# Madhudorai/encodec-pytorch

Measured on AMD Instinct MI355X. Metric: audio-seconds/sec EnCodec24k train step, batch 32x1s, higher is better.
Workload: dtype f32; 1 GPU; config 3: 24 kHz mono full GAN (MS-STFT disc + Balancer); global_batch=32, parallelism=dp1

## Files before the change

encodec-pytorch_amd/csrc/resblock.hip:

```cpp
#include "common.h"
#include "prof.h"

namespace {

typedef float f32x4v __attribute__((ext_vector_type(4)));
ENCX_DEV f32x4v mfma16(float a, float b, f32x4v c) { return __builtin_amdgcn_mfma_f32_16x16x4f32(a, b, c, 0, 0, 0); }

constexpr int TT = 64;
constexpr int XF = 80;
constexpr int XW = 67;

template <int C>
struct Rb {
    static constexpr int HD = C / 2;
    static constexpr int CG = C == 64 ? 2 : 1;
    static constexpr int NT = 256 * CG;
    static constexpr int SLAB = C * C + C * HD + HD * 3 * C + C + HD;
};

struct RbArgs {
    const float* x;
    const float* w1;
    const float* b1;
    const float* w2;
    const float* b2;
    const float* ws;
    const float* bs;
    float* h;
    float* y;
    const float* dy;
    float* dx;
    float* dh;
    float* slab;
    int B, T, NT;
};

ENCX_DEV void st4(float* row, int t, int T, f32x4v v) {
    if (t + 4 <= T) {
        *(f32x4u*)(row + t) = (f32x4u){v[0], v[1], v[2], v[3]};
    } else {
#pragma unroll
        for (int i = 0; i < 4; ++i)
            if (t + i < T) row[t + i] = v[i];
    }
}
ENCX_DEV f32x4v ld4(const float* row, int t, int T) {
    if (t + 4 <= T) return ld4u(row + t);
    f32x4v v;
#pragma unroll
    for (int i = 0; i < 4; ++i) v[i] = t + i < T ? row[t + i] : 0.f;
    return v;
}
ENCX_DEV int reflect_clamp(int t, int T) { return t < 0 ? -t : (t < T ? t : T - 1); }
typedef __amdgpu_buffer_rsrc_t rsrc_t;
ENCX_DEV rsrc_t rsrc(const float* base, int64_t n) {
    return __builtin_amdgcn_make_buffer_rsrc((void*)base, (short)0, (int)(n * sizeof(float)), 0x00020000);
}
ENCX_DEV float bload(rsrc_t r, int voff, int soff) {
    return __builtin_bit_cast(float, __builtin_amdgcn_raw_buffer_load_b32(r, voff, soff, 0));
}

template <int C>
__global__ __launch_bounds__(Rb<C>::NT) void rb_fwd_kernel(RbArgs a) {
    constexpr int HD = C / 2, CG = Rb<C>::CG, NT = Rb<C>::NT, N1 = HD / 16 / CG, N2 = C / 16 / CG;
    extern __shared__ float sm[];
    float* xs = sm;
    float* es = xs + C * XF;
    float* hs = es + C * XF;
    const int tid = threadIdx.x, lane = tid & 63, wv = tid >> 6, lc = lane & 15, lk = lane >> 4;
    const int m0 = 16 * (wv & 3), g = wv >> 2;
    float bw1[3][C / 4][N1], bw2[HD / 4][N2], bws[C / 4][N2], b1v[N1], bov[N2];
#pragma unroll
    for (int n = 0; n < N1; ++n) {
        const int j = (g * N1 + n) * 16 + lc;
        b1v[n] = a.b1[j];
#pragma unroll
        for (int k = 0; k < 3; ++k)
#pragma unroll
            for (int c4 = 0; c4 < C / 4; ++c4) bw1[k][c4][n] = a.w1[((4 * c4 + lk) * 3 + k) * HD + j];
    }
#pragma unroll
    for (int n = 0; n < N2; ++n) {
        const int o = (g * N2 + n) * 16 + lc;
        bov[n] = a.b2[o] + a.bs[o];
#pragma unroll
        for (int j4 = 0; j4 < HD / 4; ++j4) bw2[j4][n] = a.w2[(4 * j4 + lk) * C + o];
#pragma unroll
        for (int c4 = 0; c4 < C / 4; ++c4) bws[c4][n] = a.ws[(4 * c4 + lk) * C + o];
    }
    const int T = a.T, ntiles = a.B * a.NT;
    constexpr int NW = NT / 64, PR = C / NW;
    float pf[PR], pfh = 0.f;
    const int hc = tid >> 1, hp = TT + (tid & 1);
    auto fetch = [&](int tile) {
        const int b = tile / a.NT, t0 = (tile - b * a.NT) * TT;
        const rsrc_t rx = rsrc(a.x + (int64_t)b * C * T, (int64_t)C * T);
        const int vo = (wv * T + reflect_clamp(t0 - 2 + lane, T)) * 4;
#pragma unroll
        for (int u = 0; u < PR; ++u) pf[u] = bload(rx, vo, u * NW * T * 4);
        if (tid < 2 * C) pfh = bload(rx, (hc * T + reflect_clamp(t0 - 2 + hp, T)) * 4, 0);
    };
    if ((int)blockIdx.x < ntiles) fetch(blockIdx.x);
    for (int tile = blockIdx.x; tile < ntiles; tile += gridDim.x) {
        const int b = tile / a.NT, t0 = (tile - b * a.NT) * TT;
        __syncthreads();
#pragma unroll
        for (int u = 0; u < PR; ++u) {
            xs[(wv + NW * u) * XF + lane] = pf[u];
            es[(wv + NW * u) * XF + lane] = elu(pf[u]);
        }
        if (tid < 2 * C) {
            xs[hc * XF + hp] = pfh;
            es[hc * XF + hp] = elu(pfh);
        }
        __syncthreads();
        if (tile + (int)gridDim.x < ntiles) fetch(tile + gridDim.x);
        f32x4v acc1[N1];
#pragma unroll
        for (int n = 0; n < N1; ++n) acc1[n] = (f32x4v){0.f, 0.f, 0.f, 0.f};
#pragma unroll
        for (int k = 0; k < 3; ++k)
#pragma unroll
            for (int c4 = 0; c4 < C / 4; ++c4) {
                const float av = es[(4 * c4 + lk) * XF + m0 + lc + k];
#pragma unroll
                for (int n = 0; n < N1; ++n) acc1[n] = mfma16(av, bw1[k][c4][n], acc1[n]);
            }
        const int tq = t0 + m0 + 4 * lk;
#pragma unroll
        for (int n = 0; n < N1; ++n) {
            const int j = (g * N1 + n) * 16 + lc;
            f32x4v hv, ev;
#pragma unroll
            for (int i = 0; i < 4; ++i) {
                hv[i] = acc1[n][i] + b1v[n];
                ev[i] = elu(hv[i]);
            }
            *(f32x4v*)(hs + j * XF + m0 + 4 * lk) = ev;
            if (a.h) st4(a.h + ((int64_t)b * HD + j) * T, tq, T, hv);
        }
        __syncthreads();
        f32x4v acc2[N2];
#pragma unroll
        for (int n = 0; n < N2; ++n) acc2[n] = (f32x4v){0.f, 0.f, 0.f, 0.f};
#pragma unroll
        for (int j4 = 0; j4 < HD / 4; ++j4) {
            const float av = hs[(4 * j4 + lk) * XF + m0 + lc];
#pragma unroll
            for (int n = 0; n < N2; ++n) acc2[n] = mfma16(av, bw2[j4][n], acc2[n]);
        }
#pragma unroll
        for (int c4 = 0; c4 < C / 4; ++c4) {
            const float av = xs[(4 * c4 + lk) * XF + m0 + lc + 2];
#pragma unroll
            for (int n = 0; n < N2; ++n) acc2[n] = mfma16(av, bws[c4][n], acc2[n]);
        }
#pragma unroll
        for (int n = 0; n < N2; ++n) {
            const int o = (g * N2 + n) * 16 + lc;
            st4(a.y + ((int64_t)b * C + o) * T, tq, T, acc2[n] + bov[n]);
        }
    }
}

template <int C>
__global__ __launch_bounds__(Rb<C>::NT) void rb_dgrad_kernel(RbArgs a) {
    constexpr int HD = C / 2, CG = Rb<C>::CG, NT = Rb<C>::NT, NH = HD / 16 / CG, NX = C / 16 / CG;
    constexpr int TPO = NT / (2 * HD), U = C / TPO;
    static_assert(TPO == 8, "halo reduction assumes 8 lanes per output");
    extern __shared__ float sm[];
    float* dys = sm;
    float* dhs = dys + C * XF;
    const int tid = threadIdx.x, lane = tid & 63, wv = tid >> 6, lc = lane & 15, lk = lane >> 4;
    const int m0 = 16 * (wv & 3), g = wv >> 2;
    float bh[C / 4][NH], bs[C / 4][NX], b3[3][HD / 4][NX];
#pragma unroll
    for (int n = 0; n < NH; ++n) {
        const int j = (g * NH + n) * 16 + lc;
#pragma unroll
        for (int o4 = 0; o4 < C / 4; ++o4) bh[o4][n] = a.w2[j * C + 4 * o4 + lk];
    }
#pragma unroll
    for (int n = 0; n < NX; ++n) {
        const int c = (g * NX + n) * 16 + lc;
#pragma unroll
        for (int o4 = 0; o4 < C / 4; ++o4) bs[o4][n] = a.ws[c * C + 4 * o4 + lk];
#pragma unroll
        for (int k = 0; k < 3; ++k)
#pragma unroll
            for (int j4 = 0; j4 < HD / 4; ++j4) b3[k][j4][n] = a.w1[(c * 3 + k) * HD + 4 * j4 + lk];
    }
    const int hq = tid / TPO, hr = tid - hq * TPO, hj = hq >> 1, hp = TT + (hq & 1);
    float hw[U];
#pragma unroll
    for (int u = 0; u < U; ++u) hw[u] = a.w2[hj * C + hr * U + u];
    const int T = a.T, ntiles = a.B * a.NT;
    constexpr int NW = NT / 64, PR = C / NW;
    float pf[PR], pfh = 0.f, hh = 0.f;
    const int hc = tid >> 1, hpp = TT + (tid & 1);
    f32x4v hv[NH], xv[NX];
    auto fetch = [&](int tile) {
        const int b = tile / a.NT, t0 = (tile - b * a.NT) * TT, t = t0 + lane;
        const rsrc_t rdy = rsrc(a.dy + (int64_t)b * C * T, (int64_t)C * T);
        const int vo = (wv * T + (t < T ? t : T - 1)) * 4;
#pragma unroll
        for (int u = 0; u < PR; ++u) {
            const float v = bload(rdy, vo, u * NW * T * 4);
            pf[u] = t < T ? v : 0.f;
        }
        if (tid < 2 * C) {
            const int th = t0 + hpp;
            const float v = bload(rdy, (hc * T + (th < T ? th : T - 1)) * 4, 0);
            pfh = th < T ? v : 0.f;
        }
        const int tq = t0 + m0 + 4 * lk;
#pragma unroll
        for (int n = 0; n < NH; ++n) hv[n] = ld4(a.h + ((int64_t)b * HD + (g * NH + n) * 16 + lc) * T, tq, T);
#pragma unroll
        for (int n = 0; n < NX; ++n) xv[n] = ld4(a.x + ((int64_t)b * C + (g * NX + n) * 16 + lc) * T, tq, T);
        const int th = t0 + hp;
        hh = a.h[((int64_t)b * HD + hj) * T + (th < T ? th : T - 1)];
    };
    if ((int)blockIdx.x < ntiles) fetch(blockIdx.x);
    for (int tile = blockIdx.x; tile < ntiles; tile += gridDim.x) {
        const int b = tile / a.NT, t0 = (tile - b * a.NT) * TT;
        __syncthreads();
#pragma unroll
        for (int u = 0; u < PR; ++u) dys[(wv + NW * u) * XF + lane] = pf[u];
        if (tid < 2 * C) dys[hc * XF + hpp] = pfh;
        __syncthreads();
        const int tq = t0 + m0 + 4 * lk;
        f32x4v hcur[NH], xcur[NX];
#pragma unroll
        for (int n = 0; n < NH; ++n) hcur[n] = hv[n];
#pragma unroll
        for (int n = 0; n < NX; ++n) xcur[n] = xv[n];
        const float hhcur = hh;
        if (tile + (int)gridDim.x < ntiles) fetch(tile + gridDim.x);
        {
            f32x4v acc[NH];
#pragma unroll
            for (int n = 0; n < NH; ++n) acc[n] = (f32x4v){0.f, 0.f, 0.f, 0.f};
#pragma unroll
            for (int o4 = 0; o4 < C / 4; ++o4) {
                const float av = dys[(4 * o4 + lk) * XF + m0 + lc];
#pragma unroll
                for (int n = 0; n < NH; ++n) acc[n] = mfma16(av, bh[o4][n], acc[n]);
            }
#pragma unroll
            for (int n = 0; n < NH; ++n) {
                const int j = (g * NH + n) * 16 + lc;
                f32x4v d;
#pragma unroll
                for (int i = 0; i < 4; ++i) d[i] = tq + i < T ? acc[n][i] * elu_grad(hcur[n][i]) : 0.f;
                *(f32x4v*)(dhs + j * XF + m0 + 4 * lk) = d;
                st4(a.dh + ((int64_t)b * HD + j) * T, tq, T, d);
            }
        }
        {
            float s = 0.f;
#pragma unroll
            for (int u = 0; u < U; ++u) s = fmaf(dys[(hr * U + u) * XF + hp], hw[u], s);
            s += __shfl_xor(s, 4, 64);
            s += __shfl_xor(s, 2, 64);
            s += __shfl_xor(s, 1, 64);
            if (hr == 0) {
                const int t = t0 + hp;
                dhs[hj * XF + hp] = t < T ? s * elu_grad(hhcur) : 0.f;
            }
        }
        __syncthreads();
        f32x4v asc[NX], ak3[NX];
#pragma unroll
        for (int n = 0; n < NX; ++n) asc[n] = ak3[n] = (f32x4v){0.f, 0.f, 0.f, 0.f};
#pragma unroll
        for (int o4 = 0; o4 < C / 4; ++o4) {
            const float av = dys[(4 * o4 + lk) * XF + m0 + lc];
#pragma unroll
            for (int n = 0; n < NX; ++n) asc[n] = mfma16(av, bs[o4][n], asc[n]);
        }
#pragma unroll
        for (int k = 0; k < 3; ++k)
#pragma unroll
            for (int j4 = 0; j4 < HD / 4; ++j4) {
                const float av = dhs[(4 * j4 + lk) * XF + m0 + lc + 2 - k];
#pragma unroll
                for (int n = 0; n < NX; ++n) ak3[n] = mfma16(av, b3[k][j4][n], ak3[n]);
            }
        if (t0 == 0 && m0 == 0 && lk == 0) {
#pragma unroll
            for (int n = 0; n < NX; ++n) {
                const int c = (g * NX + n) * 16 + lc;
                float v1 = 0.f, v2 = 0.f;
#pragma unroll 1
                for (int j = 0; j < HD; ++j) {
                    const float w0 = a.w1[(c * 3) * HD + j], w1v = a.w1[(c * 3 + 1) * HD + j];
                    v1 = fmaf(w0, dhs[j * XF + 1], fmaf(w1v, dhs[j * XF + 0], v1));
                    v2 = fmaf(w0, dhs[j * XF + 0], v2);
                }
                ak3[n][1] += v1;
                ak3[n][2] += v2;
            }
        }
#pragma unroll
        for (int n = 0; n < NX; ++n) {
            const int c = (g * NX + n) * 16 + lc;
            f32x4v v;
#pragma unroll
            for (int i = 0; i < 4; ++i) v[i] = asc[n][i] + elu_grad(xcur[n][i]) * ak3[n][i];
            st4(a.dx + ((int64_t)b * C + c) * T, tq, T, v);
        }
    }
}

struct WTile {
    const float* bp;
    int kind;
    int ro, co, k;
};

template <int NTL>
ENCX_DEV void wgemm(const float* ap, const WTile* t, f32x16* acc) {
#pragma unroll 4
    for (int q = 0; q < TT; q += 2) {
        const float av = ap[q];
#pragma unroll
        for (int i = 0; i < NTL; ++i) acc[i] = mfma32(av, t[i].bp[q], acc[i]);
    }
}

template <int C>
__global__ __launch_bounds__(256) void rb_wgrad_kernel(RbArgs a) {
    constexpr int HD = C / 2, NTL = C == 64 ? 3 : 2;
    extern __shared__ float sm[];
    float* dys = sm;
    float* dhs = dys + C * XW;
    float* hes = dhs + HD * XW;
    float* xs = hes + HD * XW;
    float* exs = xs + C * XW;
    const int tid = threadIdx.x, lane = tid & 63, wv = tid >> 6, lr = lane & 31, lq = lane >> 5;
    const int lh = lr & (HD - 1);
    const float* ap;
    WTile tl[NTL];
    int ntl = NTL;
    if (C == 64) {
        if (wv < 2) {
            ap = dys + (32 * wv + lr) * XW;
            tl[0] = {xs + lr * XW + 2, 0, 32 * wv, 0, 0};
            tl[1] = {xs + (32 + lr) * XW + 2, 0, 32 * wv, 32, 0};
            tl[2] = {hes + lh * XW, 1, 32 * wv, 0, 0};
        } else {
            ap = dhs + lh * XW;
#pragma unroll
            for (int i = 0; i < 3; ++i) {
                const int u = 3 * (wv - 2) + i, k = u >> 1, co = 32 * (u & 1);
                tl[i] = {exs + (co + lr) * XW + k, 2, 0, co, k};
            }
        }
    } else {
        if (wv == 0) {
            ap = dys + lr * XW;
            tl[0] = {xs + lr * XW + 2, 0, 0, 0, 0};
            tl[1] = {hes + lh * XW, 1, 0, 0, 0};
        } else {
            ap = dhs + lh * XW;
            tl[0] = {exs + lr * XW + (wv - 1), 2, 0, 0, wv - 1};
            tl[1] = tl[0];
            ntl = 1;
        }
    }
    ap += lq;
#pragma unroll
    for (int i = 0; i < NTL; ++i) tl[i].bp += lq;
    f32x16 acc[NTL];
#pragma unroll
    for (int i = 0; i < NTL; ++i)
#pragma unroll
        for (int r = 0; r < 16; ++r) acc[i][r] = 0.f;
    const int T = a.T, ntiles = a.B * a.NT;
    constexpr int PD = C / 4, PH = HD / 4;
    float pd[PD], pdh[PH], ph[PH], px[PD], pxh = 0.f;
    float bacc[PD + PH];
#pragma unroll
    for (int u = 0; u < PD + PH; ++u) bacc[u] = 0.f;
    const int hc = tid >> 1, hp = TT + (tid & 1);
    auto fetch = [&](int tile) {
        const int b = tile / a.NT, t0 = (tile - b * a.NT) * TT, t = t0 + lane;
        const rsrc_t rdy = rsrc(a.dy + (int64_t)b * C * T, (int64_t)C * T);
        const rsrc_t rdh = rsrc(a.dh + (int64_t)b * HD * T, (int64_t)HD * T);
        const rsrc_t rh = rsrc(a.h + (int64_t)b * HD * T, (int64_t)HD * T);
        const rsrc_t rx = rsrc(a.x + (int64_t)b * C * T, (int64_t)C * T);
        const int vo = (wv * T + (t < T ? t : T - 1)) * 4, vx = (wv * T + reflect_clamp(t0 - 2 + lane, T)) * 4;
#pragma unroll
        for (int u = 0; u < PD; ++u) {
            const float v = bload(rdy, vo, u * 4 * T * 4);
            pd[u] = t < T ? v : 0.f;
            px[u] = bload(rx, vx, u * 4 * T * 4);
        }
#pragma unroll
        for (int u = 0; u < PH; ++u) {
            const float v = bload(rdh, vo, u * 4 * T * 4);
            pdh[u] = t < T ? v : 0.f;
            ph[u] = bload(rh, vo, u * 4 * T * 4);
        }
        if (tid < 2 * C) pxh = bload(rx, (hc * T + reflect_clamp(t0 - 2 + hp, T)) * 4, 0);
    };
    if ((int)blockIdx.x < ntiles) fetch(blockIdx.x);
    for (int tile = blockIdx.x; tile < ntiles; tile += gridDim.x) {
        __syncthreads();
#pragma unroll
        for (int u = 0; u < PD; ++u) {
            dys[(wv + 4 * u) * XW + lane] = pd[u];
            xs[(wv + 4 * u) * XW + lane] = px[u];
            exs[(wv + 4 * u) * XW + lane] = elu(px[u]);
            bacc[u] += pd[u];
        }
#pragma unroll
        for (int u = 0; u < PH; ++u) {
            dhs[(wv + 4 * u) * XW + lane] = pdh[u];
            hes[(wv + 4 * u) * XW + lane] = elu(ph[u]);
            bacc[PD + u] += pdh[u];
        }
        if (tid < 2 * C) {
            xs[hc * XW + hp] = pxh;
            exs[hc * XW + hp] = elu(pxh);
        }
        __syncthreads();
        if (tile + (int)gridDim.x < ntiles) fetch(tile + gridDim.x);
        if (C == 64 || ntl == NTL) wgemm<NTL>(ap, tl, acc);
        else wgemm<1>(ap, tl, acc);
    }
    float* sl = a.slab + (int64_t)blockIdx.x * Rb<C>::SLAB;
#pragma unroll
    for (int i = 0; i < NTL; ++i) {
        if (i >= ntl) break;
        const WTile& t = tl[i];
#pragma unroll
        for (int r = 0; r < 16; ++r) {
            const int row = t.ro + mfma_row(r, lane), col = t.co + lr;
            if (t.kind == 0) sl[row * C + col] = acc[i][r];
            else if (t.kind == 1) {
                if (col < HD) sl[C * C + row * HD + col] = acc[i][r];
            } else if (row < HD) {
                sl[C * C + C * HD + (row * C + col) * 3 + t.k] = acc[i][r];
            }
        }
    }
#pragma unroll
    for (int u = 0; u < PD + PH; ++u) {
        const float v = wave_sum(bacc[u]);
        if (lane == 0) sl[C * C + C * HD + HD * 3 * C + (u < PD ? wv + 4 * u : C + wv + 4 * (u - PD))] = v;
    }
}

template <int C>
__global__ __launch_bounds__(256) void rb_wgrad_reduce(const float* slab, int G, float* dws, float* dw2, float* dw1,
                                                       float* db2, float* dbs, float* db1, int acc_w, int acc_b) {
    constexpr int HD = C / 2, S = Rb<C>::SLAB;
    __shared__ double red[256];
    const int64_t i = (int64_t)blockIdx.x * 64 + (threadIdx.x & 63);
    const bool valid = i < S;
    const float v = slab_sum_256_d(slab + (valid ? i : 0), G, S, valid, red);
    if (threadIdx.x >= 64 || !valid) return;
    auto put = [](float* p, float v, int acc) {
        if (p) *p = acc ? *p + v : v;
    };
    int k = (int)i;
    if (k < C * C) { put(dws ? dws + k : nullptr, v, acc_w); return; }
    k -= C * C;
    if (k < C * HD) { put(dw2 ? dw2 + k : nullptr, v, acc_w); return; }
    k -= C * HD;
    if (k < HD * 3 * C) { put(dw1 ? dw1 + k : nullptr, v, acc_w); return; }
    k -= HD * 3 * C;
    if (k < C) {
        put(db2 ? db2 + k : nullptr, v, acc_b);
        put(dbs ? dbs + k : nullptr, v, acc_b);
        return;
    }
    k -= C;
    put(db1 ? db1 + k : nullptr, v, acc_b);
}

size_t rb_fwd_lds(int C) { return (size_t)(2 * C + C / 2) * XF * sizeof(float); }
size_t rb_dgrad_lds(int C) { return (size_t)(C + C / 2) * XF * sizeof(float); }
size_t rb_wgrad_lds(int C) { return (size_t)(3 * C + C) * XW * sizeof(float); }

int num_cus() {
    static int n = 0;
    if (!n) {
        int dev = 0;
        if (hipGetDevice(&dev) != hipSuccess ||
            hipDeviceGetAttribute(&n, hipDeviceAttributeMultiprocessorCount, dev) != hipSuccess || n <= 0)
            n = 256;
    }
    return n;
}
template <typename K>
int rb_grid(K kernel, int threads, size_t lds, int64_t tiles) {
    int per_cu = 0;
    if (hipOccupancyMaxActiveBlocksPerMultiprocessor(&per_cu, kernel, threads, lds) != hipSuccess || per_cu < 1)
        per_cu = 1;
    const int64_t g = (int64_t)per_cu * num_cus();
    return (int)(tiles < g ? tiles : g);
}
bool rb_ok(int64_t C, int64_t T) { return (C == 32 || C == 64) && T >= 3; }

template <int C>
int rb_wgrad_grid(int64_t tiles) {
    static int g = 0;
    if (!g) g = rb_grid(rb_wgrad_kernel<C>, 256, rb_wgrad_lds(C), (int64_t)1 << 40);
    return (int)(tiles < g ? tiles : g);
}

template <int C>
void launch_bwd(const RbArgs& a, float* dws, float* dw2, float* dw1, float* db2, float* dbs, float* db1, int acc_w,
                int acc_b, hipStream_t st) {
    const int64_t tiles = (int64_t)a.B * a.NT;
    static int gd = 0;
    if (!gd) gd = rb_grid(rb_dgrad_kernel<C>, Rb<C>::NT, rb_dgrad_lds(C), (int64_t)1 << 40);
    hipLaunchKernelGGL((rb_dgrad_kernel<C>), dim3((unsigned)(tiles < gd ? tiles : gd)), dim3(Rb<C>::NT),
                       rb_dgrad_lds(C), st, a);
    const int gw = rb_wgrad_grid<C>(tiles);
    hipLaunchKernelGGL((rb_wgrad_kernel<C>), dim3(gw), dim3(256), rb_wgrad_lds(C), st, a);
    hipLaunchKernelGGL(rb_wgrad_reduce<C>, dim3((unsigned)cdiv(Rb<C>::SLAB, 64)), dim3(256), 0, st, a.slab, gw, dws,
                       dw2, dw1, db2, dbs, db1, acc_w, acc_b);
}

template <int C>
void launch_fwd(const RbArgs& a, int64_t tiles, hipStream_t st) {
    static int g = 0;
    if (!g) g = rb_grid(rb_fwd_kernel<C>, Rb<C>::NT, rb_fwd_lds(C), (int64_t)1 << 40);
    hipLaunchKernelGGL((rb_fwd_kernel<C>), dim3((unsigned)(tiles < g ? tiles : g)), dim3(Rb<C>::NT), rb_fwd_lds(C),
                       st, a);
}

}

extern "C" {

int encx_resblock_fwd(const float* x, const float* w1, const float* b1, const float* w2, const float* b2,
                      const float* ws, const float* bs, float* h, float* y, int64_t B, int64_t C, int64_t T,
                      encx_stream_t stream) {
    ENCX_REQUIRE(x && w1 && b1 && w2 && b2 && ws && bs && y && B > 0 && rb_ok(C, T));
    hipStream_t st = (hipStream_t)stream;
    const int64_t HD = C / 2;
    encx_prof_scope ps(st, 2.0 * B * T * (3 * C * HD + (HD + C) * C), 4.0 * B * T * (2 * C + HD), "conv_rb_fwd");
    ps.tag(" C%ld T%ld", (long)C, (long)T);
    RbArgs a{x, w1, b1, w2, b2, ws, bs, h, y, nullptr, nullptr, nullptr, nullptr, (int)B, (int)T, (int)cdiv(T, TT)};
    const int64_t tiles = B * a.NT;
    if (C == 32) launch_fwd<32>(a, tiles, st);
    else launch_fwd<64>(a, tiles, st);
    ENCX_CHECK_LAUNCH();
    return 0;
}

size_t encx_resblock_bwd_workspace(int64_t B, int64_t C, int64_t T) {
    if (!rb_ok(C, T) || B <= 0) return 0;
    const int64_t tiles = B * cdiv(T, TT);
    const size_t slab = C == 32 ? (size_t)rb_wgrad_grid<32>(tiles) * Rb<32>::SLAB
                                : (size_t)rb_wgrad_grid<64>(tiles) * Rb<64>::SLAB;
    return ((size_t)B * (C / 2) * T + slab) * sizeof(float);
}

int encx_resblock_bwd(const float* dy, const float* x, const float* h, const float* w1, const float* w2,
                      const float* ws, float* dx, float* dw1, float* db1, float* dw2, float* db2, float* dws,
                      float* dbs, int acc_w, int acc_b, float* wsp, int64_t B, int64_t C, int64_t T,
                      encx_stream_t stream) {
    ENCX_REQUIRE(dy && x && h && w1 && w2 && ws && dx && wsp && B > 0 && rb_ok(C, T));
    hipStream_t st = (hipStream_t)stream;
    const int64_t HD = C / 2;
    encx_prof_scope ps(st, 4.0 * B * T * (3 * C * HD + (HD + C) * C), 4.0 * B * T * (4 * C + 2 * HD), "conv_rb_bwd");
    ps.tag(" C%ld T%ld", (long)C, (long)T);
    float* dh = wsp;
    float* slab = wsp + (size_t)B * HD * T;
    RbArgs a{x, w1, nullptr, w2, nullptr, ws, nullptr, const_cast<float*>(h), nullptr, dy, dx, dh, slab, (int)B, (int)T,
             (int)cdiv(T, TT)};
    if (C == 32) launch_bwd<32>(a, dws, dw2, dw1, db2, dbs, db1, acc_w, acc_b, st);
    else launch_bwd<64>(a, dws, dw2, dw1, db2, dbs, db1, acc_w, acc_b, st);
    ENCX_CHECK_LAUNCH();
    return 0;
}

}
```

include/encx.h:

```cpp
#ifndef ENCX_H
#define ENCX_H

#include <stddef.h>
#include <stdint.h>

#ifdef __cplusplus
extern "C" {
#endif

typedef struct ihipStream_t* encx_stream_t;

#define ENCX_OK 0
#define ENCX_EINVAL 9001

#define ENCX_PAD_ZERO 0
#define ENCX_PAD_REFLECT 1
#define ENCX_ACT_NONE 0
#define ENCX_ACT_ELU 1

int encx_version(void);
const char* encx_build_id(void);
const char* encx_strerror(int code);
int encx_option_count(void);
const char* encx_option_name(int i);
int encx_get_option(const char* name, int64_t* value);
int encx_set_option(const char* name, int64_t value, int64_t* previous );
int encx_blas_stats(int64_t* launched, int64_t* declined);
int encx_init(int device);
int encx_prof_enable(int on);
int encx_prof_enabled(void);
int encx_prof_read(double* total_ms, double* total_flops, double* total_bytes, int64_t* launches);
int encx_prof_slot(int64_t i, double* ms, double* flops, double* bytes, const char** tag);

int encx_weightnorm_fwd(const float* v, const float* g, float* wf, float* wp, int64_t A0,
                        int64_t A1, int64_t K, int64_t stride, encx_stream_t stream);
int encx_weightnorm_bwd(const float* v, const float* g, const float* dw, float* dv, float* dg,
                        int64_t rows, int64_t cols, int accumulate, encx_stream_t stream);
typedef struct {
    const float* v; const float* g; float* wf; float* wp;
    int64_t A0, A1, K, stride, row0;
} encx_wn_fwd_desc;
typedef struct {
    const float* v; const float* g; const float* dw; float* dv; float* dg;
    int64_t rows, cols, row0, accumulate;
} encx_wn_bwd_desc;
int encx_weightnorm_fwd_batch(const encx_wn_fwd_desc* layers, int64_t n_layers, int64_t rows_total,
                              encx_stream_t stream);
int encx_weightnorm_bwd_batch(const encx_wn_bwd_desc* layers, int64_t n_layers, int64_t rows_total,
                              encx_stream_t stream);

size_t encx_conv1d_fwd_workspace(int64_t B, int64_t Cin, int64_t Cout, int64_t Tout, int64_t K,
                                 int64_t stride, int64_t dilation);
int encx_conv1d_fwd(const float* x, const float* wf, const float* bias, const float* residual,
                    float* y, float* ws, int64_t B, int64_t Cin, int64_t Tin, int64_t Cout,
                    int64_t Tout, int64_t K, int64_t stride, int64_t dilation, int64_t pad_left,
                    int64_t short_ext, int pad_mode, int pre_act, encx_stream_t stream);
size_t encx_conv1d_bwd_data_workspace(int64_t B, int64_t Cin, int64_t Tin, int64_t Cout,
                                      int64_t Tout, int64_t K, int64_t stride, int64_t pad_left,
                                      int64_t pad_right);
int encx_conv1d_bwd_data(const float* dy, const float* wp, const float* x, float* dx, float* ws,
                         int64_t B, int64_t Cin, int64_t Tin, int64_t Cout, int64_t Tout,
                         int64_t K, int64_t stride, int64_t pad_left, int64_t pad_right,
                         int64_t short_ext, int pad_mode, int pre_act, int accumulate,
                         encx_stream_t stream);
int encx_conv1d_bwd_data_dilated(const float* dy, const float* wf, const float* x, float* dx, float* ws,
                                 int64_t B, int64_t Cin, int64_t Tin, int64_t Cout, int64_t Tout,
                                 int64_t K, int64_t stride, int64_t dilation, int64_t pad_left,
                                 int64_t pad_right, int64_t short_ext, int pad_mode, int pre_act,
                                 int accumulate, encx_stream_t stream);
int encx_conv1d_bwd_weight(const float* dy, const float* x, float* dw, float* db, float* ws,
                           int64_t B, int64_t Cin, int64_t Tin, int64_t Cout, int64_t Tout,
                           int64_t K, int64_t stride, int64_t dilation, int64_t pad_left,
                           int64_t short_ext, int pad_mode, int pre_act, int accumulate,
                           encx_stream_t stream);
int encx_conv1d_bwd_weight_bias(const float* dy, const float* x, float* dw, float* db, float* ws, int64_t B,
                                int64_t Cin, int64_t Tin, int64_t Cout, int64_t Tout, int64_t K, int64_t stride,
                                int64_t dilation, int64_t pad_left, int64_t short_ext, int pad_mode, int pre_act,
                                int acc_w, int acc_b, encx_stream_t stream);
size_t encx_conv1d_bwd_weight_workspace(int64_t B, int64_t Cin, int64_t Cout, int64_t Tout,
                                        int64_t K);

size_t encx_convtr1d_fwd_workspace(int64_t B, int64_t Cin, int64_t Cout, int64_t Tout, int64_t K,
                                   int64_t stride, int64_t trim_left);
int encx_convtr1d_fwd(const float* x, const float* wp, const float* bias, float* y, float* ws,
                      int64_t B, int64_t Cin, int64_t Tin, int64_t Cout, int64_t Tout, int64_t K,
                      int64_t stride, int64_t trim_left, int pre_act, encx_stream_t stream);
size_t encx_convtr1d_bwd_data_workspace(int64_t B, int64_t Cin, int64_t Tin, int64_t Cout,
                                        int64_t K, int64_t stride);
int encx_convtr1d_bwd_data(const float* dy, const float* wf, const float* x, float* dx, float* ws,
                           int64_t B, int64_t Cin, int64_t Tin, int64_t Cout, int64_t Tout,
                           int64_t K, int64_t stride, int64_t trim_left, int pre_act,
                           int accumulate, encx_stream_t stream);
int encx_convtr1d_bwd_weight(const float* x, const float* dy, float* dw, float* db, float* ws,
                             int64_t B, int64_t Cin, int64_t Tin, int64_t Cout, int64_t Tout,
                             int64_t K, int64_t stride, int64_t trim_left, int pre_act,
                             int accumulate, encx_stream_t stream);
size_t encx_convtr1d_bwd_weight_workspace(int64_t B, int64_t Cin, int64_t Cout, int64_t Tin,
                                          int64_t K);

int encx_resblock_fwd(const float* x, const float* w1, const float* b1, const float* w2, const float* b2,
                      const float* ws, const float* bs, float* h, float* y, int64_t B, int64_t C, int64_t T,
                      encx_stream_t stream);
size_t encx_resblock_bwd_workspace(int64_t B, int64_t C, int64_t T);
int encx_resblock_bwd(const float* dy, const float* x, const float* h, const float* w1, const float* w2,
                      const float* ws, float* dx, float* dw1, float* db1, float* dw2, float* db2, float* dws,
                      float* dbs, int acc_w, int acc_b, float* wsp, int64_t B, int64_t C, int64_t T,
                      encx_stream_t stream);

size_t encx_channel_sum_workspace(int64_t C);
int encx_channel_sum(const float* dy, float* db, float* ws, int64_t B, int64_t C, int64_t T,
                     int accumulate, encx_stream_t stream);
int encx_normalize_fwd(const float* x, float* xn, float* scale, int64_t B, int64_t C, int64_t T,
                       encx_stream_t stream);
int encx_scale_rows(const float* x, const float* scale, float* y, int64_t B, int64_t CT,
                    encx_stream_t stream);
int encx_axpby(const float* x, float* y, int64_t n, float alpha, const float* alpha_dev,
               float beta, encx_stream_t stream);
int encx_l1_loss(const float* x, const float* y, float* loss, float* grad, float* ws, int64_t n,
                 encx_stream_t stream);

int encx_rvq_argmin(const float* res, const float* embed, int64_t* idx, uint64_t* keys,
                    int64_t B, int64_t D, int64_t Tf, int64_t Kc, int direct,
                    encx_stream_t stream);
int encx_rvq_apply(const float* x, float* res_out, const float* embed, const int64_t* idx,
                   float* out, float* commit_dir, float* commit_part, int64_t B, int64_t D,
                   int64_t Tf, int first, int ste, encx_stream_t stream);
int encx_rvq_gather(const float* embed, const int64_t* idx, float* out, int64_t B, int64_t D,
                    int64_t Tf, int accumulate, encx_stream_t stream);
int64_t encx_rvq_apply_parts(int64_t B, int64_t D, int64_t Tf);
size_t encx_rvq_bucket_workspace(int64_t N, int64_t D, int64_t Kc);
int encx_rvq_ema(const float* x, const int64_t* idx, float* cluster_size, float* embed_avg,
                 float* embed, float* ws, int64_t B, int64_t D, int64_t Tf, int64_t Kc,
                 float decay, float eps, encx_stream_t stream);
int encx_rvq_code_sums(const float* x, const int64_t* idx, float* sums, float* ws, int64_t B,
                       int64_t D, int64_t Tf, int64_t Kc, encx_stream_t stream);
int encx_rvq_ema_from_sums(const float* sums, float* cluster_size, float* embed_avg, float* embed,
                           int64_t D, int64_t Kc, float decay, float eps, encx_stream_t stream);
int encx_kmeans_step(const float* samples, float* means, int64_t* bins, int64_t* idx,
                     uint64_t* keys, float* ws, int64_t N, int64_t D, int64_t Kc,
                     encx_stream_t stream);
int encx_sample_rows(const float* samples, float* out, int64_t N, int64_t D, int64_t num,
                     uint64_t seed, encx_stream_t stream);
int encx_bdt_to_nd(const float* res, float* out, int64_t B, int64_t D, int64_t Tf,
                   encx_stream_t stream);
int encx_reduce_sum(const float* parts, int64_t n, float scale, float* out, int accumulate,
                    encx_stream_t stream);

size_t encx_mel_tables_floats(int64_t n_fft, int64_t n_mels);
int encx_spec_tables_window(float* tables, const float* window, int64_t n_fft, encx_stream_t stream);
int encx_mel_tables_init(float* tables, const float* mel_basis, int64_t n_fft, int64_t n_mels,
                         encx_stream_t stream);
size_t encx_mel_workspace_floats(int64_t B, int64_t T, int64_t n_fft, int64_t n_mels);
int encx_mel_loss(const float* x, const float* y, const float* tables, float* ws, float* loss,
                  float* grad, int64_t B, int64_t T, int64_t n_fft, int64_t n_mels,
                  encx_stream_t stream);

size_t encx_mel_loss_multi_workspace_floats(int64_t B, int64_t T, const int64_t* n_ffts, int64_t nscales);
int encx_mel_loss_multi(const float* x, const float* y, const float* const* tables, const int64_t* n_ffts,
                        int64_t nscales, float* ws, float* loss, float* grad, int64_t B, int64_t T,
                        encx_stream_t stream);
int encx_mel_logmel(const float* x, const float* tables, float* ws, float* out, int64_t B,
                    int64_t T, int64_t n_fft, int64_t n_mels, encx_stream_t stream);
int64_t encx_mel_frames(int64_t T, int64_t n_fft);
size_t encx_mel_logmel_framed_workspace_floats(int64_t B, int64_t T, int64_t n_fft, int64_t hop);
int encx_mel_logmel_framed(const float* x, const float* win_tables, const float* mel_basis, float* ws, float* out,
                           int64_t B, int64_t T, int64_t n_fft, int64_t hop, int64_t n_mels, encx_stream_t stream);

int encx_lincomb(const float* x, const float* z, float* out, int64_t n, float a, const float* bdev,
                 float bscale, encx_stream_t stream);
size_t encx_item_norm_workspace(int64_t B);
int encx_item_norm_mean(const float* g, float* out, float* ws, int64_t B, int64_t L,
                        encx_stream_t stream);
#define ENCX_BALANCER_MAX_LOSSES 64
int encx_balancer_update(const float* norms, double* total, double* fix, double* avg, float* red,
                         int nl, double beta, float count, encx_stream_t stream);
int encx_balancer_scales(const double* avg, const float* red, const double* ratio, float* scales,
                         int nl, double total_norm, double eps, int from_red,
                         encx_stream_t stream);
int encx_balancer_combine(const float* g0, const float* g1, const float* g2, const float* g3,
                          const float* scales, float* out, int64_t n, encx_stream_t stream);
int encx_adam_step(float* p, const float* g, float* m, float* v, int64_t n, double lr, double beta1,
                   double beta2, double eps, int64_t step, encx_stream_t stream);
int encx_adam_hyper(float* hp, double lr, double beta1, double beta2, double eps, int64_t step,
                    encx_stream_t stream);
int encx_adam_step_dev(float* p, const float* g, float* m, float* v, int64_t n, const float* hp,
                       encx_stream_t stream);
// ... 265 lines not shown
```

Baseline: 983.2 audio-seconds/sec.

## Fuse resblock data-grad and weight-grad kernels into one backward kernel

Merges the separate dgrad and wgrad resblock backward kernels into a single persistent kernel. dh is now computed in LDS and consumed directly by the weight-gradient GEMM instead of being written to and re-read from global memory, and dy/x/h tiles are loaded once for both uses. For C=64 the block has two wave groups, so the time axis of the weight GEMM is split across them and their partial results are reduced through LDS. Some weights move to LDS to limit register pressure. This removes a launch and a global round-trip of dh, at the cost of more LDS per block, which may lower occupancy.

```diff
diff --git a/encodec-pytorch_amd/csrc/resblock.hip b/encodec-pytorch_amd/csrc/resblock.hip
--- a/encodec-pytorch_amd/csrc/resblock.hip
+++ b/encodec-pytorch_amd/csrc/resblock.hip
@@ -30,7 +30,6 @@
     float* y;
     const float* dy;
     float* dx;
-    float* dh;
     float* slab;
     int B, T, NT;
 };
@@ -43,13 +42,6 @@
         for (int i = 0; i < 4; ++i)
             if (t + i < T) row[t + i] = v[i];
     }
-}
-ENCX_DEV f32x4v ld4(const float* row, int t, int T) {
-    if (t + 4 <= T) return ld4u(row + t);
-    f32x4v v;
-#pragma unroll
-    for (int i = 0; i < 4; ++i) v[i] = t + i < T ? row[t + i] : 0.f;
-    return v;
 }
 ENCX_DEV int reflect_clamp(int t, int T) { return t < 0 ? -t : (t < T ? t : T - 1); }
 typedef __amdgpu_buffer_rsrc_t rsrc_t;
@@ -163,166 +155,16 @@
     }
 }
 
-template <int C>
-__global__ __launch_bounds__(Rb<C>::NT) void rb_dgrad_kernel(RbArgs a) {
-    constexpr int HD = C / 2, CG = Rb<C>::CG, NT = Rb<C>::NT, NH = HD / 16 / CG, NX = C / 16 / CG;
-    constexpr int TPO = NT / (2 * HD), U = C / TPO;
-    static_assert(TPO == 8, "halo reduction assumes 8 lanes per output");
-    extern __shared__ float sm[];
-    float* dys = sm;
-    float* dhs = dys + C * XF;
-    const int tid = threadIdx.x, lane = tid & 63, wv = tid >> 6, lc = lane & 15, lk = lane >> 4;
-    const int m0 = 16 * (wv & 3), g = wv >> 2;
-    float bh[C / 4][NH], bs[C / 4][NX], b3[3][HD / 4][NX];
-#pragma unroll
-    for (int n = 0; n < NH; ++n) {
-        const int j = (g * NH + n) * 16 + lc;
-#pragma unroll
-        for (int o4 = 0; o4 < C / 4; ++o4) bh[o4][n] = a.w2[j * C + 4 * o4 + lk];
-    }
-#pragma unroll
-    for (int n = 0; n < NX; ++n) {
-        const int c = (g * NX + n) * 16 + lc;
-#pragma unroll
-        for (int o4 = 0; o4 < C / 4; ++o4) bs[o4][n] = a.ws[c * C + 4 * o4 + lk];
-#pragma unroll
-        for (int k = 0; k < 3; ++k)
-#pragma unroll
-            for (int j4 = 0; j4 < HD / 4; ++j4) b3[k][j4][n] = a.w1[(c * 3 + k) * HD + 4 * j4 + lk];
-    }
-    const int hq = tid / TPO, hr = tid - hq * TPO, hj = hq >> 1, hp = TT + (hq & 1);
-    float hw[U];
-#pragma unroll
-    for (int u = 0; u < U; ++u) hw[u] = a.w2[hj * C + hr * U + u];
-    const int T = a.T, ntiles = a.B * a.NT;
-    constexpr int NW = NT / 64, PR = C / NW;
-    float pf[PR], pfh = 0.f, hh = 0.f;
-    const int hc = tid >> 1, hpp = TT + (tid & 1);
-    f32x4v hv[NH], xv[NX];
-    auto fetch = [&](int tile) {
-        const int b = tile / a.NT, t0 = (tile - b * a.NT) * TT, t = t0 + lane;
-        const rsrc_t rdy = rsrc(a.dy + (int64_t)b * C * T, (int64_t)C * T);
-        const int vo = (wv * T + (t < T ? t : T - 1)) * 4;
-#pragma unroll
-        for (int u = 0; u < PR; ++u) {
-            const float v = bload(rdy, vo, u * NW * T * 4);
-            pf[u] = t < T ? v : 0.f;
-        }
-        if (tid < 2 * C) {
-            const int th = t0 + hpp;
-            const float v = bload(rdy, (hc * T + (th < T ? th : T - 1)) * 4, 0);
-            pfh = th < T ? v : 0.f;
-        }
-        const int tq = t0 + m0 + 4 * lk;
-#pragma unroll
-        for (int n = 0; n < NH; ++n) hv[n] = ld4(a.h + ((int64_t)b * HD + (g * NH + n) * 16 + lc) * T, tq, T);
-#pragma unroll
-        for (int n = 0; n < NX; ++n) xv[n] = ld4(a.x + ((int64_t)b * C + (g * NX + n) * 16 + lc) * T, tq, T);
-        const int th = t0 + hp;
-        hh = a.h[((int64_t)b * HD + hj) * T + (th < T ? th : T - 1)];
-    };
-    if ((int)blockIdx.x < ntiles) fetch(blockIdx.x);
-    for (int tile = blockIdx.x; tile < ntiles; tile += gridDim.x) {
-        const int b = tile / a.NT, t0 = (tile - b * a.NT) * TT;
-        __syncthreads();
-#pragma unroll
-        for (int u = 0; u < PR; ++u) dys[(wv + NW * u) * XF + lane] = pf[u];
-        if (tid < 2 * C) dys[hc * XF + hpp] = pfh;
-        __syncthreads();
-        const int tq = t0 + m0 + 4 * lk;
-        f32x4v hcur[NH], xcur[NX];
-#pragma unroll
-        for (int n = 0; n < NH; ++n) hcur[n] = hv[n];
-#pragma unroll
-        for (int n = 0; n < NX; ++n) xcur[n] = xv[n];
-        const float hhcur = hh;
-        if (tile + (int)gridDim.x < ntiles) fetch(tile + gridDim.x);
-        {
-            f32x4v acc[NH];
-#pragma unroll
-            for (int n = 0; n < NH; ++n) acc[n] = (f32x4v){0.f, 0.f, 0.f, 0.f};
-#pragma unroll
-            for (int o4 = 0; o4 < C / 4; ++o4) {
-                const float av = dys[(4 * o4 + lk) * XF + m0 + lc];
-#pragma unroll
-                for (int n = 0; n < NH; ++n) acc[n] = mfma16(av, bh[o4][n], acc[n]);
-            }
-#pragma unroll
-            for (int n = 0; n < NH; ++n) {
-                const int j = (g * NH + n) * 16 + lc;
-                f32x4v d;
-#pragma unroll
-                for (int i = 0; i < 4; ++i) d[i] = tq + i < T ? acc[n][i] * elu_grad(hcur[n][i]) : 0.f;
-                *(f32x4v*)(dhs + j * XF + m0 + 4 * lk) = d;
-                st4(a.dh + ((int64_t)b * HD + j) * T, tq, T, d);
-            }
-        }
-        {
-            float s = 0.f;
-#pragma unroll
-            for (int u = 0; u < U; ++u) s = fmaf(dys[(hr * U + u) * XF + hp], hw[u], s);
-            s += __shfl_xor(s, 4, 64);
-            s += __shfl_xor(s, 2, 64);
-            s += __shfl_xor(s, 1, 64);
-            if (hr == 0) {
-                const int t = t0 + hp;
-                dhs[hj * XF + hp] = t < T ? s * elu_grad(hhcur) : 0.f;
-            }
-        }
-        __syncthreads();
-        f32x4v asc[NX], ak3[NX];
-#pragma unroll
-        for (int n = 0; n < NX; ++n) asc[n] = ak3[n] = (f32x4v){0.f, 0.f, 0.f, 0.f};
-#pragma unroll
-        for (int o4 = 0; o4 < C / 4; ++o4) {
-            const float av = dys[(4 * o4 + lk) * XF + m0 + lc];
-#pragma unroll
-            for (int n = 0; n < NX; ++n) asc[n] = mfma16(av, bs[o4][n], asc[n]);
-        }
-#pragma unroll
-        for (int k = 0; k < 3; ++k)
-#pragma unroll
-            for (int j4 = 0; j4 < HD / 4; ++j4) {
-                const float av = dhs[(4 * j4 + lk) * XF + m0 + lc + 2 - k];
-#pragma unroll
-                for (int n = 0; n < NX; ++n) ak3[n] = mfma16(av, b3[k][j4][n], ak3[n]);
-            }
-        if (t0 == 0 && m0 == 0 && lk == 0) {
-#pragma unroll
-            for (int n = 0; n < NX; ++n) {
-                const int c = (g * NX + n) * 16 + lc;
-                float v1 = 0.f, v2 = 0.f;
-#pragma unroll 1
-                for (int j = 0; j < HD; ++j) {
-                    const float w0 = a.w1[(c * 3) * HD + j], w1v = a.w1[(c * 3 + 1) * HD + j];
-                    v1 = fmaf(w0, dhs[j * XF + 1], fmaf(w1v, dhs[j * XF + 0], v1));
-                    v2 = fmaf(w0, dhs[j * XF + 0], v2);
-                }
-                ak3[n][1] += v1;
-                ak3[n][2] += v2;
-            }
-        }
-#pragma unroll
-        for (int n = 0; n < NX; ++n) {
-            const int c = (g * NX + n) * 16 + lc;
-            f32x4v v;
-#pragma unroll
-            for (int i = 0; i < 4; ++i) v[i] = asc[n][i] + elu_grad(xcur[n][i]) * ak3[n][i];
-            st4(a.dx + ((int64_t)b * C + c) * T, tq, T, v);
-        }
-    }
-}
-
 struct WTile {
     const float* bp;
     int kind;
     int ro, co, k;
 };
 
-template <int NTL>
+template <int NTL, int QN>
 ENCX_DEV void wgemm(const float* ap, const WTile* t, f32x16* acc) {
 #pragma unroll 4
-    for (int q = 0; q < TT; q += 2) {
+    for (int q = 0; q < QN; q += 2) {
         const float av = ap[q];
 #pragma unroll
         for (int i = 0; i < NTL; ++i) acc[i] = mfma32(av, t[i].bp[q], acc[i]);
@@ -330,126 +172,271 @@
 }
 
 template <int C>
-__global__ __launch_bounds__(256) void rb_wgrad_kernel(RbArgs a) {
-    constexpr int HD = C / 2, NTL = C == 64 ? 3 : 2;
+__global__ __launch_bounds__(Rb<C>::NT) void rb_bwd_kernel(RbArgs a) {
+    constexpr int HD = C / 2, CG = Rb<C>::CG, NT = Rb<C>::NT, NH = HD / 16 / CG, NX = C / 16 / CG;
+    constexpr int TPO = NT / (2 * HD), U = C / TPO;
+    constexpr int NTL = C == 64 ? 3 : 2, QN = TT / CG;
+    static_assert(TPO == 8, "halo reduction assumes 8 lanes per output");
     extern __shared__ float sm[];
-    float* dys = sm;
+    float* dyp = sm;
+    float* dhp = dyp + C * XF;
+    float* dys = dhp + HD * XF;
     float* dhs = dys + C * XW;
-    float* hes = dhs + HD * XW;
+    float* hs = dhs + HD * XW;
+    float* hes = hs + HD * XW;
     float* xs = hes + HD * XW;
     float* exs = xs + C * XW;
-    const int tid = threadIdx.x, lane = tid & 63, wv = tid >> 6, lr = lane & 31, lq = lane >> 5;
+    constexpr bool WL = C == 64;
+    float* w3s = exs + C * XW;
+    float* hws = w3s + 3 * (HD / 4) * NX * CG * 64;
+    const int tid = threadIdx.x, lane = tid & 63, wv = tid >> 6, lc = lane & 15, lk = lane >> 4;
+    const int m0 = 16 * (wv & 3), g = wv >> 2;
+    float bh[C / 4][NH], bs[C / 4][NX], b3[WL ? 1 : 3][HD / 4][NX];
+#pragma unroll
+    for (int n = 0; n < NH; ++n) {
+        const int j = (g * NH + n) * 16 + lc;
+#pragma unroll
+        for (int o4 = 0; o4 < C / 4; ++o4) bh[o4][n] = a.w2[j * C + 4 * o4 + lk];
+    }
+#pragma unroll
+    for (int n = 0; n < NX; ++n) {
+        const int c = (g * NX + n) * 16 + lc;
+#pragma unroll
+        for (int o4 = 0; o4 < C / 4; ++o4) bs[o4][n] = a.ws[c * C + 4 * o4 + lk];
+#pragma unroll
+        for (int k = 0; k < 3; ++k)
+#pragma unroll
+            for (int j4 = 0; j4 < HD / 4; ++j4) {
+                const float w = a.w1[(c * 3 + k) * HD + 4 * j4 + lk];
+                if (!WL) b3[k][j4][n] = w;
+                else if (m0 == 0) w3s[(((k * (HD / 4) + j4) * NX + n) * CG + g) * 64 + lane] = w;
+            }
+    }
+    const int hq = tid / TPO, hr = tid - hq * TPO, hj = hq >> 1, hp = TT + (hq & 1);
+    const int hwi = hj * TPO + hr;
+    float hw[WL ? 1 : U];
+#pragma unroll
+    for (int u = 0; u < U; ++u) {
+        const float w = a.w2[hj * C + hr * U + u];
+        if (!WL) hw[u] = w;
+        else if (!(hq & 1)) hws[u * (NT / 2) + hwi] = w;
+    }
+    auto w3 = [&](int k, int j4, int n) {
+        return WL ? w3s[(((k * (HD / 4) + j4) * NX + n) * CG + g) * 64 + lane] : b3[WL ? 0 : k][j4][n];
+    };
+    const int lr = lane & 31, lq = lane >> 5, wr = wv & 3;
     const int lh = lr & (HD - 1);
     const float* ap;
     WTile tl[NTL];
     int ntl = NTL;
     if (C == 64) {
-        if (wv < 2) {
-            ap = dys + (32 * wv + lr) * XW;
-            tl[0] = {xs + lr * XW + 2, 0, 32 * wv, 0, 0};
-            tl[1] = {xs + (32 + lr) * XW + 2, 0, 32 * wv, 32, 0};
-            tl[2] = {hes + lh * XW, 1, 32 * wv, 0, 0};
+        if (wr < 2) {
+            ap = dys + (32 * wr + lr) * XW;
+            tl[0] = {xs + lr * XW + 2, 0, 32 * wr, 0, 0};
+            tl[1] = {xs + (32 + lr) * XW + 2, 0, 32 * wr, 32, 0};
+            tl[2] = {hes + lh * XW, 1, 32 * wr, 0, 0};
         } else {
             ap = dhs + lh * XW;
 #pragma unroll
             for (int i = 0; i < 3; ++i) {
-                const int u = 3 * (wv - 2) + i, k = u >> 1, co = 32 * (u & 1);
+                const int u = 3 * (wr - 2) + i, k = u >> 1, co = 32 * (u & 1);
                 tl[i] = {exs + (co + lr) * XW + k, 2, 0, co, k};
             }
         }
     } else {
-        if (wv == 0) {
+        if (wr == 0) {
             ap = dys + lr * XW;
             tl[0] = {xs + lr * XW + 2, 0, 0, 0, 0};
             tl[1] = {hes + lh * XW, 1, 0, 0, 0};
         } else {
             ap = dhs + lh * XW;
-            tl[0] = {exs + lr * XW + (wv - 1), 2, 0, 0, wv - 1};
+            tl[0] = {exs + lr * XW + (wr - 1), 2, 0, 0, wr - 1};
             tl[1] = tl[0];
             ntl = 1;
         }
     }
-    ap += lq;
-#pragma unroll
-    for (int i = 0; i < NTL; ++i) tl[i].bp += lq;
+    const int qo = lq + QN * g;
+    ap += qo;
+#pragma unroll
+    for (int i = 0; i < NTL; ++i) tl[i].bp += qo;
     f32x16 acc[NTL];
 #pragma unroll
     for (int i = 0; i < NTL; ++i)
 #pragma unroll
         for (int r = 0; r < 16; ++r) acc[i][r] = 0.f;
     const int T = a.T, ntiles = a.B * a.NT;
-    constexpr int PD = C / 4, PH = HD / 4;
-    float pd[PD], pdh[PH], ph[PH], px[PD], pxh = 0.f;
+    constexpr int NW = NT / 64, PD = C / NW, PH = HD / NW;
+    float pd[PD], px[PD], ph[PH], pdh = 0.f, pxh = 0.f, phh = 0.f;
     float bacc[PD + PH];
 #pragma unroll
     for (int u = 0; u < PD + PH; ++u) bacc[u] = 0.f;
-    const int hc = tid >> 1, hp = TT + (tid & 1);
+    const int hc = tid >> 1, hpp = TT + (tid & 1);
     auto fetch = [&](int tile) {
-        const int b = tile / a.NT, t0 = (tile - b * a.NT) * TT, t = t0 + lane;
+        const int b = tile / a.NT, t0 = (tile - b * a.NT) * TT, t = t0 + lane, th = t0 + hpp;
         const rsrc_t rdy = rsrc(a.dy + (int64_t)b * C * T, (int64_t)C * T);
-        const rsrc_t rdh = rsrc(a.dh + (int64_t)b * HD * T, (int64_t)HD * T);
         const rsrc_t rh = rsrc(a.h + (int64_t)b * HD * T, (int64_t)HD * T);
         const rsrc_t rx = rsrc(a.x + (int64_t)b * C * T, (int64_t)C * T);
         const int vo = (wv * T + (t < T ? t : T - 1)) * 4, vx = (wv * T + reflect_clamp(t0 - 2 + lane, T)) * 4;
 #pragma unroll
         for (int u = 0; u < PD; ++u) {
-            const float v = bload(rdy, vo, u * 4 * T * 4);
+            const float v = bload(rdy, vo, u * NW * T * 4);
             pd[u] = t < T ? v : 0.f;
-            px[u] = bload(rx, vx, u * 4 * T * 4);
-        }
-#pragma unroll
-        for (int u = 0; u < PH; ++u) {
-            const float v = bload(rdh, vo, u * 4 * T * 4);
-            pdh[u] = t < T ? v : 0.f;
-            ph[u] = bload(rh, vo, u * 4 * T * 4);
-        }
-        if (tid < 2 * C) pxh = bload(rx, (hc * T + reflect_clamp(t0 - 2 + hp, T)) * 4, 0);
+            px[u] = bload(rx, vx, u * NW * T * 4);
+        }
+#pragma unroll
+        for (int u = 0; u < PH; ++u) ph[u] = bload(rh, vo, u * NW * T * 4);
+        if (tid < 2 * C) {
+            const float v = bload(rdy, (hc * T + (th < T ? th : T - 1)) * 4, 0);
+            pdh = th < T ? v : 0.f;
+            pxh = bload(rx, (hc * T + reflect_clamp(t0 - 2 + hpp, T)) * 4, 0);
+        }
+        if (tid < 2 * HD) phh = bload(rh, (hc * T + (th < T ? th : T - 1)) * 4, 0);
     };
     if ((int)blockIdx.x < ntiles) fetch(blockIdx.x);
     for (int tile = blockIdx.x; tile < ntiles; tile += gridDim.x) {
+        const int b = tile / a.NT, t0 = (tile - b * a.NT) * TT;
         __syncthreads();
 #pragma unroll
         for (int u = 0; u < PD; ++u) {
-            dys[(wv + 4 * u) * XW + lane] = pd[u];
-            xs[(wv + 4 * u) * XW + lane] = px[u];
-            exs[(wv + 4 * u) * XW + lane] = elu(px[u]);
+            const int r = wv + NW * u;
+            dyp[r * XF + lane] = pd[u];
+            dys[r * XW + lane] = pd[u];
+            xs[r * XW + lane] = px[u];
+            exs[r * XW + lane] = elu(px[u]);
             bacc[u] += pd[u];
         }
 #pragma unroll
         for (int u = 0; u < PH; ++u) {
-            dhs[(wv + 4 * u) * XW + lane] = pdh[u];
-            hes[(wv + 4 * u) * XW + lane] = elu(ph[u]);
-            bacc[PD + u] += pdh[u];
+            const int r = wv + NW * u;
+            hs[r * XW + lane] = ph[u];
+            hes[r * XW + lane] = elu(ph[u]);
         }
         if (tid < 2 * C) {
-            xs[hc * XW + hp] = pxh;
-            exs[hc * XW + hp] = elu(pxh);
-        }
+            dyp[hc * XF + hpp] = pdh;
+            xs[hc * XW + hpp] = pxh;
+            exs[hc * XW + hpp] = elu(pxh);
+        }
+        if (tid < 2 * HD) hs[hc * XW + hpp] = phh;
         __syncthreads();
         if (tile + (int)gridDim.x < ntiles) fetch(tile + gridDim.x);
-        if (C == 64 || ntl == NTL) wgemm<NTL>(ap, tl, acc);
-        else wgemm<1>(ap, tl, acc);
+        const int pq = m0 + 4 * lk, tq = t0 + pq;
+        {
+            f32x4v ah[NH];
+#pragma unroll
+            for (int n = 0; n < NH; ++n) ah[n] = (f32x4v){0.f, 0.f, 0.f, 0.f};
+#pragma unroll
+            for (int o4 = 0; o4 < C / 4; ++o4) {
+                const float av = dyp[(4 * o4 + lk) * XF + m0 + lc];
+#pragma unroll
+                for (int n = 0; n < NH; ++n) ah[n] = mfma16(av, bh[o4][n], ah[n]);
+            }
+#pragma unroll
+            for (int n = 0; n < NH; ++n) {
+                const int j = (g * NH + n) * 16 + lc;
+                f32x4v d;
+#pragma unroll
+                for (int i = 0; i < 4; ++i) {
+                    d[i] = tq + i < T ? ah[n][i] * elu_grad(hs[j * XW + pq + i]) : 0.f;
+                    dhs[j * XW + pq + i] = d[i];
+                }
+                *(f32x4v*)(dhp + j * XF + pq) = d;
+            }
+        }
+        {
+            float s = 0.f;
+#pragma unroll
+            for (int u = 0; u < U; ++u) s = fmaf(dyp[(hr * U + u) * XF + hp], WL ? hws[u * (NT / 2) + hwi] : hw[WL ? 0 : u], s);
+            s += __shfl_xor(s, 4, 64);
+            s += __shfl_xor(s, 2, 64);
+            s += __shfl_xor(s, 1, 64);
+            if (hr == 0) dhp[hj * XF + hp] = t0 + hp < T ? s * elu_grad(hs[hj * XW + hp]) : 0.f;
+        }
+        __syncthreads();
+        {
+            f32x4v asc[NX], ak3[NX];
+#pragma unroll
+            for (int n = 0; n < NX; ++n) asc[n] = ak3[n] = (f32x4v){0.f, 0.f, 0.f, 0.f};
+#pragma unroll
+            for (int o4 = 0; o4 < C / 4; ++o4) {
+                const float av = dyp[(4 * o4 + lk) * XF + m0 + lc];
+#pragma unroll
+                for (int n = 0; n < NX; ++n) asc[n] = mfma16(av, bs[o4][n], asc[n]);
+            }
+#pragma unroll
+            for (int k = 0; k < 3; ++k)
+#pragma unroll
+                for (int j4 = 0; j4 < HD / 4; ++j4) {
+                    const float av = dhp[(4 * j4 + lk) * XF + m0 + lc + 2 - k];
+#pragma unroll
+                    for (int n = 0; n < NX; ++n) ak3[n] = mfma16(av, w3(k, j4, n), ak3[n]);
+                }
+            if (t0 == 0 && m0 == 0 && lk == 0) {
+#pragma unroll
+                for (int n = 0; n < NX; ++n) {
+                    const int c = (g * NX + n) * 16 + lc;
+                    float v1 = 0.f, v2 = 0.f;
+#pragma unroll 1
+                    for (int j = 0; j < HD; ++j) {
+                        const float w0 = a.w1[(c * 3) * HD + j], w1v = a.w1[(c * 3 + 1) * HD + j];
+                        v1 = fmaf(w0, dhp[j * XF + 1], fmaf(w1v, dhp[j * XF + 0], v1));
+                        v2 = fmaf(w0, dhp[j * XF + 0], v2);
+                    }
+                    ak3[n][1] += v1;
+                    ak3[n][2] += v2;
+                }
+            }
+#pragma unroll
+            for (int n = 0; n < NX; ++n) {
+                const int c = (g * NX + n) * 16 + lc;
+                f32x4v v;
+#pragma unroll
+                for (int i = 0; i < 4; ++i) v[i] = asc[n][i] + elu_grad(xs[c * XW + pq + i + 2]) * ak3[n][i];
+                st4(a.dx + ((int64_t)b * C + c) * T, tq, T, v);
+            }
+        }
+        if (C == 64 || ntl == NTL) wgemm<NTL, QN>(ap, tl, acc);
+        else wgemm<1, QN>(ap, tl, acc);
+#pragma unroll
+        for (int u = 0; u < PH; ++u) bacc[PD + u] += dhs[(wv + NW * u) * XW + lane];
+    }
+    if (CG == 2) {
+        __syncthreads();
+        if (g == 1) {
+#pragma unroll
+            for (int i = 0; i < NTL; ++i)
+#pragma unroll
+                for (int r = 0; r < 16; ++r) sm[((wr * NTL + i) * 16 + r) * 64 + lane] = acc[i][r];
+        }
+        __syncthreads();
+        if (g == 0) {
+#pragma unroll
+            for (int i = 0; i < NTL; ++i)
+#pragma unroll
+                for (int r = 0; r < 16; ++r) acc[i][r] += sm[((wr * NTL + i) * 16 + r) * 64 + lane];
+        }
     }
     float* sl = a.slab + (int64_t)blockIdx.x * Rb<C>::SLAB;
-#pragma unroll
-    for (int i = 0; i < NTL; ++i) {
-        if (i >= ntl) break;
-        const WTile& t = tl[i];
-#pragma unroll
-        for (int r = 0; r < 16; ++r) {
-            const int row = t.ro + mfma_row(r, lane), col = t.co + lr;
-            if (t.kind == 0) sl[row * C + col] = acc[i][r];
-            else if (t.kind == 1) {
-                if (col < HD) sl[C * C + row * HD + col] = acc[i][r];
-            } else if (row < HD) {
-                sl[C * C + C * HD + (row * C + col) * 3 + t.k] = acc[i][r];
+    if (g == 0) {
+#pragma unroll
+        for (int i = 0; i < NTL; ++i) {
+            if (i >= ntl) break;
+            const WTile& t = tl[i];
+#pragma unroll
+            for (int r = 0; r < 16; ++r) {
+                const int row = t.ro + mfma_row(r, lane), col = t.co + lr;
+                if (t.kind == 0) sl[row * C + col] = acc[i][r];
+                else if (t.kind == 1) {
+                    if (col < HD) sl[C * C + row * HD + col] = acc[i][r];
+                } else if (row < HD) {
+                    sl[C * C + C * HD + (row * C + col) * 3 + t.k] = acc[i][r];
+                }
             }
         }
     }
 #pragma unroll
     for (int u = 0; u < PD + PH; ++u) {
         const float v = wave_sum(bacc[u]);
-        if (lane == 0) sl[C * C + C * HD + HD * 3 * C + (u < PD ? wv + 4 * u : C + wv + 4 * (u - PD))] = v;
+        if (lane == 0) sl[C * C + C * HD + HD * 3 * C + (u < PD ? wv + NW * u : C + wv + NW * (u - PD))] = v;
     }
 }
 
@@ -482,8 +469,9 @@
 }
 
 size_t rb_fwd_lds(int C) { return (size_t)(2 * C + C / 2) * XF * sizeof(float); }
-size_t rb_dgrad_lds(int C) { return (size_t)(C + C / 2) * XF * sizeof(float); }
-size_t rb_wgrad_lds(int C) { return (size_t)(3 * C + C) * XW * sizeof(float); }
+size_t rb_bwd_lds(int C) {
+    return (size_t)((C + C / 2) * XF + (3 * C + 3 * (C / 2)) * XW + (C == 64 ? 3 * C * (C / 2) + (C / 2) * C : 0)) * sizeof(float);
+}
 
 int num_cus() {
     static int n = 0;
@@ -506,23 +494,19 @@
 bool rb_ok(int64_t C, int64_t T) { return (C == 32 || C == 64) && T >= 3; }
 
 template <int C>
-int rb_wgrad_grid(int64_t tiles) {
+int rb_bwd_grid() {
     static int g = 0;
-    if (!g) g = rb_grid(rb_wgrad_kernel<C>, 256, rb_wgrad_lds(C), (int64_t)1 << 40);
-    return (int)(tiles < g ? tiles : g);
+    if (!g) g = rb_grid(rb_bwd_kernel<C>, Rb<C>::NT, rb_bwd_lds(C), (int64_t)1 << 40);
+    return g;
 }
 
 template <int C>
 void launch_bwd(const RbArgs& a, float* dws, float* dw2, float* dw1, float* db2, float* dbs, float* db1, int acc_w,
                 int acc_b, hipStream_t st) {
     const int64_t tiles = (int64_t)a.B * a.NT;
-    static int gd = 0;
-    if (!gd) gd = rb_grid(rb_dgrad_kernel<C>, Rb<C>::NT, rb_dgrad_lds(C), (int64_t)1 << 40);
-    hipLaunchKernelGGL((rb_dgrad_kernel<C>), dim3((unsigned)(tiles < gd ? tiles : gd)), dim3(Rb<C>::NT),
-                       rb_dgrad_lds(C), st, a);
-    const int gw = rb_wgrad_grid<C>(tiles);
-    hipLaunchKernelGGL((rb_wgrad_kernel<C>), dim3(gw), dim3(256), rb_wgrad_lds(C), st, a);
-    hipLaunchKernelGGL(rb_wgrad_reduce<C>, dim3((unsigned)cdiv(Rb<C>::SLAB, 64)), dim3(256), 0, st, a.slab, gw, dws,
+    const int gd = (int)std::min<int64_t>(tiles, rb_bwd_grid<C>());
+    hipLaunchKernelGGL((rb_bwd_kernel<C>), dim3(gd), dim3(Rb<C>::NT), rb_bwd_lds(C), st, a);
+    hipLaunchKernelGGL(rb_wgrad_reduce<C>, dim3((unsigned)cdiv(Rb<C>::SLAB, 64)), dim3(256), 0, st, a.slab, gd, dws,
                        dw2, dw1, db2, dbs, db1, acc_w, acc_b);
 }
 
@@ -546,7 +530,7 @@
     const int64_t HD = C / 2;
     encx_prof_scope ps(st, 2.0 * B * T * (3 * C * HD + (HD + C) * C), 4.0 * B * T * (2 * C + HD), "conv_rb_fwd");
     ps.tag(" C%ld T%ld", (long)C, (long)T);
-    RbArgs a{x, w1, b1, w2, b2, ws, bs, h, y, nullptr, nullptr, nullptr, nullptr, (int)B, (int)T, (int)cdiv(T, TT)};
+    RbArgs a{x, w1, b1, w2, b2, ws, bs, h, y, nullptr, nullptr, nullptr, (int)B, (int)T, (int)cdiv(T, TT)};
     const int64_t tiles = B * a.NT;
     if (C == 32) launch_fwd<32>(a, tiles, st);
     else launch_fwd<64>(a, tiles, st);
@@ -554,12 +538,12 @@
     return 0;
 }
 
+int encx_resblock_bwd_grid(int64_t C) { return C == 32 ? rb_bwd_grid<32>() : C == 64 ? rb_bwd_grid<64>() : 0; }
+
 size_t encx_resblock_bwd_workspace(int64_t B, int64_t C, int64_t T) {
     if (!rb_ok(C, T) || B <= 0) return 0;
-    const int64_t tiles = B * cdiv(T, TT);
-    const size_t slab = C == 32 ? (size_t)rb_wgrad_grid<32>(tiles) * Rb<32>::SLAB
-                                : (size_t)rb_wgrad_grid<64>(tiles) * Rb<64>::SLAB;
-    return ((size_t)B * (C / 2) * T + slab) * sizeof(float);
+    const int64_t tiles = B * cdiv(T, TT), g = std::min<int64_t>(tiles, encx_resblock_bwd_grid(C));
+    return (size_t)g * (C == 32 ? Rb<32>::SLAB : Rb<64>::SLAB) * sizeof(float);
 }
 
 int encx_resblock_bwd(const float* dy, const float* x, const float* h, const float* w1, const float* w2,
@@ -569,11 +553,9 @@
     ENCX_REQUIRE(dy && x && h && w1 && w2 && ws && dx && wsp && B > 0 && rb_ok(C, T));
     hipStream_t st = (hipStream_t)stream;
     const int64_t HD = C / 2;
-    encx_prof_scope ps(st, 4.0 * B * T * (3 * C * HD + (HD + C) * C), 4.0 * B * T * (4 * C + 2 * HD), "conv_rb_bwd");
+    encx_prof_scope ps(st, 4.0 * B * T * (3 * C * HD + (HD + C) * C), 4.0 * B * T * (3 * C + HD), "conv_rb_bwd");
     ps.tag(" C%ld T%ld", (long)C, (long)T);
-    float* dh = wsp;
-    float* slab = wsp + (size_t)B * HD * T;
-    RbArgs a{x, w1, nullptr, w2, nullptr, ws, nullptr, const_cast<float*>(h), nullptr, dy, dx, dh, slab, (int)B, (int)T,
+    RbArgs a{x, w1, nullptr, w2, nullptr, ws, nullptr, const_cast<float*>(h), nullptr, dy, dx, wsp, (int)B, (int)T,
              (int)cdiv(T, TT)};
     if (C == 32) launch_bwd<32>(a, dws, dw2, dw1, db2, dbs, db1, acc_w, acc_b, st);
     else launch_bwd<64>(a, dws, dw2, dw1, db2, dbs, db1, acc_w, acc_b, st);
diff --git a/include/encx.h b/include/encx.h
--- a/include/encx.h
+++ b/include/encx.h
@@ -102,6 +102,7 @@
                       const float* ws, const float* bs, float* h, float* y, int64_t B, int64_t C, int64_t T,
                       encx_stream_t stream);
 size_t encx_resblock_bwd_workspace(int64_t B, int64_t C, int64_t T);
+int encx_resblock_bwd_grid(int64_t C);
 int encx_resblock_bwd(const float* dy, const float* x, const float* h, const float* w1, const float* w2,
                       const float* ws, float* dx, float* dw1, float* db1, float* dw2, float* db2, float* dws,
                       float* dbs, int acc_w, int acc_b, float* wsp, int64_t B, int64_t C, int64_t T,
```

After: 983.1 audio-seconds/sec, median of 3. About the same (-0.0%).
